# pbenner/kmerLr

Hardware: NVIDIA B200
Metric: kmer_sequences_per_sec (higher is better)
Workload: dtype f64

## Files before the change

kmerlr_b200/csrc/abi.cu:

```cuda
#include <cmath>
#include <map>
#include <mutex>
#include <unordered_map>
#include <vector>

#include "common.cuh"

namespace kl {

namespace {
Ctx g_ctx;
std::mutex g_mutex;
std::unordered_map<uint64_t, std::shared_ptr<Object>> g_objects;
uint64_t g_next = 1;
thread_local std::string g_error;
}

Ctx &ctx() { return g_ctx; }

namespace {
std::multimap<size_t, void *> g_free_blocks;
std::unordered_map<void *, size_t> g_block_size;
constexpr size_t ARENA_GRAIN = (size_t)2 << 20;
}
// ... 32 lines not shown
  KL_CUDA(cudaEventSynchronize(g_ctx.staging_ev));
  if (bytes > g_ctx.staging_bytes) {
    if (g_ctx.staging) KL_CUDA(cudaFreeHost(g_ctx.staging));
    g_ctx.staging = nullptr; g_ctx.staging_bytes = 0;
    const size_t want = (bytes + ARENA_GRAIN - 1) / ARENA_GRAIN * ARENA_GRAIN;
    KL_CUDA(cudaMallocHost(&g_ctx.staging, want));
    g_ctx.staging_bytes = want;
  }
  return g_ctx.staging;
}

namespace {
struct ProfRec { std::string name; cudaEvent_t e0, e1; };
std::vector<ProfRec> g_prof_pending;
std::vector<cudaEvent_t> g_prof_pool;
std::unordered_map<std::string, std::pair<double, int64_t>> g_prof_totals;
cudaEvent_t prof_event() {
  if (!g_prof_pool.empty()) { cudaEvent_t e = g_prof_pool.back(); g_prof_pool.pop_back(); return e; }
  cudaEvent_t e;
  KL_CUDA(cudaEventCreate(&e));
  return e;
}
void prof_resolve() {
  if (g_prof_pending.empty()) return;
  KL_CUDA(cudaStreamSynchronize(g_ctx.stream));
  for (auto &r : g_prof_pending) {
    float ms = 0.f;
    KL_CUDA(cudaEventElapsedTime(&ms, r.e0, r.e1));
    auto &t = g_prof_totals[r.name];
    t.first += ms; t.second += 1;
    g_prof_pool.push_back(r.e0); g_prof_pool.push_back(r.e1);
  }
  g_prof_pending.clear();
}
}
void profile_begin(const char *name) {
  if (g_prof_pending.size() > 8192) prof_resolve();
  ProfRec r{name, prof_event(), prof_event()};
  KL_CUDA(cudaEventRecord(r.e0, g_ctx.stream));
  g_prof_pending.push_back(r);
}
void profile_end() { KL_CUDA(cudaEventRecord(g_prof_pending.back().e1, g_ctx.stream)); }

void require_ready() {
  if (!g_ctx.ready) fail(KMERLR_ERR_NOGPU, "kmerlr_init() has not succeeded: no usable sm_100 GPU (there is no CPU fallback)");
}

uint64_t register_object(std::shared_ptr<Object> o) {
  uint64_t h = g_next++;
// ... 424 lines not shown
```

kmerlr_b200/csrc/common.cuh:

```cuda
#pragma once

#include <cuda_runtime.h>
#include <stdint.h>

#include <chrono>
#include <cstdio>
#include <cstdlib>
#include <cstring>
#include <memory>
#include <string>
#include <vector>

#include "../../include/kmerlr_b200.h"

namespace kl {

struct Error {
  int code;
  std::string msg;
};

[[noreturn]] inline void fail(int code, const std::string &msg) { throw Error{code, msg}; }

#define KL_CUDA(expr)                                                                              \
  do {                                                                                             \
    cudaError_t _e = (expr);                                                                       \
    if (_e != cudaSuccess)                                                                         \
      ::kl::fail(KMERLR_ERR_CUDA, std::string(#expr) + ": " + cudaGetErrorString(_e) + " (" +      \
                                      __FILE__ + ":" + std::to_string(__LINE__) + ")");            \
  } while (0)

#define KL_REQUIRE(cond, msg)                                                                      \
  do {                                                                                             \
// ... 37 lines not shown
  cudaEvent_t copy_ev[CTX_COPY_EVENTS] = {nullptr};
  cudaEvent_t ev0 = nullptr, ev1 = nullptr;
  void *staging = nullptr;
  size_t staging_bytes = 0;
  cudaEvent_t staging_ev = nullptr;
  std::vector<std::shared_ptr<const Numbering>> numbering;
  int64_t launches = 0;
  double last_ms = 0.0;
  bool profiling = false;
  bool implicit_ok = true;
  int super_len = -1;
  int hot_cols = 6144;
  int fused_ticket = 8;
  void *comm = nullptr;
  int rank = 0, world = 1;
  PeerBox *peer = nullptr;
  bool p2p_ok = true;
  bool p2p_allreduce = false;
  int feed_growth = 135;
  int small_long = -1;
  int persist_bps = 0;
  bool coop_supported = true;
  bool coop_ok = true;
};
Ctx &ctx();
void require_ready();

void profile_begin(const char *name);
void profile_end();

#define KL_LAUNCH(kernel, grid, block, smem, ...)                                                  \
  do {                                                                                             \
    if (::kl::ctx().profiling) ::kl::profile_begin(#kernel);                                       \
    kernel<<<(grid), (block), (smem), ::kl::ctx().stream>>>(__VA_ARGS__);                          \
    if (::kl::ctx().profiling) ::kl::profile_end();                                                \
    ::kl::ctx().launches++;                                                                        \
    KL_CUDA(cudaGetLastError());                                                                   \
  } while (0)

inline void sync_stream() { KL_CUDA(cudaStreamSynchronize(ctx().stream)); }

void *host_staging(size_t bytes);
inline void host_staging_done() { KL_CUDA(cudaEventRecord(ctx().staging_ev, ctx().stream)); }

struct Trace {
  bool on;
  std::chrono::steady_clock::time_point t0, last;
  const char *what;
  explicit Trace(const char *w) : what(w) {
    static int env = -1;
    if (env < 0) { const char *e = getenv("KMERLR_TRACE"); env = (e && *e == '1') ? 1 : 0; }
    on = env == 1;
    if (on) t0 = last = std::chrono::steady_clock::now();
  }
  void mark(const char *phase, bool sync = true) {
    if (!on) return;
    if (sync) cudaStreamSynchronize(ctx().stream);
    auto t = std::chrono::steady_clock::now();
    fprintf(stderr, "[trace %s] %-28s %8.3f ms (total %8.3f)\n", what, phase,
            std::chrono::duration<double, std::milli>(t - last).count(),
            std::chrono::duration<double, std::milli>(t - t0).count());
    last = t;
  }
// ... 289 lines not shown
```

kmerlr_b200/csrc/extract.cu:

```cuda
#include <cmath>

#include "extract_kernel.cuh"

namespace kl {

namespace {

using namespace xk;

__global__ void pack_kernel(const uint8_t *__restrict__ seq, const int64_t *__restrict__ off,
                            const int64_t *__restrict__ blk, int64_t n, int64_t total_blocks, int64_t w0, int64_t w1,
                            uint32_t *__restrict__ bits2, uint16_t *__restrict__ inv16) {
  int64_t w = w0 + (int64_t)blockIdx.x * blockDim.x + threadIdx.x;
  if (w >= w1) return;
  const int64_t b = w >> 2;
  int64_t g = (int64_t)((double)b * (double)n / (double)total_blocks);
  g = g < 0 ? 0 : (g > n - 1 ? n - 1 : g);
  int64_t lo, hi, stepw = 1;
  if (blk[g] <= b) {
    lo = g; hi = g + 1;
    while (hi < n && blk[hi] <= b) { lo = hi; stepw <<= 1; hi = hi + stepw < n ? hi + stepw : n; }
  } else {
    hi = g; lo = g - 1;
    while (lo > 0 && blk[lo] > b) { hi = lo; stepw <<= 1; lo = lo - stepw > 0 ? lo - stepw : 0; }
// ... 501 lines not shown
  LI.M = cfg.M; LI.N = cfg.N; LI.op = P.op;
  for (int k = cfg.M; k <= cfg.N + 1; k++) LI.level_off[k] = P.level_off[k];
  std::shared_ptr<const Numbering> num;
  if (n_frozen > 0) {
    frozen_bits.assign((size_t)nw, 0u);
    uint64_t prev = 0;
    for (int64_t j = 0; j < n_frozen; j++) {
      int k = frozen_k[j];
      KL_REQUIRE(k >= cfg.M && k <= cfg.N && frozen_code[j] < (1ull << (2 * k)), "frozen class outside [M,N]");
      uint64_t id = (uint64_t)P.level_off[k] + frozen_code[j];
      KL_REQUIRE(j == 0 || id > prev, "frozen class list must be sorted by (k, code) without duplicates");
      prev = id;
      frozen_bits[id >> 5] |= 1u << (id & 31);
    }
    auto F = std::make_shared<Numbering>();
    F->M = cfg.M; F->N = cfg.N; F->op = P.op; F->nw = nw; F->count = (uint32_t)n_frozen;
    F->bits.alloc((size_t)nw); F->rank.alloc((size_t)nw + 1);
    F->bits.upload(frozen_bits.data(), (size_t)nw);
    number_set(*F);
    num = F;
  } else {
    num = numbering_all(LI, nw);
  }
  DevBuf<unsigned long long> tot(9);
  tot.zero();
  bitmap.zero();
  DevBuf<uint32_t> full(1);
  full.zero();
  P.full = full.p; P.nb_words = nw;
  P.st_id = out->col.p; P.st_cnt = P.binarize ? dummy_cnt.p : out->val_u32.p; P.rowcnt = out->rowcnt.p;
  P.bitmap = bitmap.p; P.nbx = num->nbx.p; P.filter = n_frozen > 0; P.stats = tot.p + 1;
  P.mark = n_frozen == 0;
  DevBuf<uint32_t> lowbits, rowdup;
  if (hybrid) {
    P.events = 1;
    P.low_words = P.t_lo <= P.t_hi ? (int)((P.tl_cnt + 31) / 32) : 0;
    if (P.low_words) { lowbits.alloc((size_t)s.n * P.low_words); P.lowbits = lowbits.p; }
    rowdup.alloc((size_t)s.n);
    P.rowdup = rowdup.p;
  }
  DevBuf<uint32_t> ovf;
  P.ovf_stride = nbl * (s.max_len > 0 ? s.max_len : 1);
  if (nbl && (!P.binarize || hybrid) && s.n > 0) {
    ovf.alloc((size_t)ctx().sm_count * 64 * (size_t)P.ovf_stride);
    P.ovf = ovf.p;
  }
  tr.mark("alloc");

  if (s.n > 0) {
    const int nchunks = feed ? feed->nchunks : 1;
    DevBuf<uint32_t> ticket((size_t)nchunks);
    ticket.zero();
    const bool two_streams = feed && nchunks > 1;
    DevBuf<uint32_t> ovf2;
    if (two_streams && P.ovf) ovf2.alloc((size_t)ctx().sm_count * 64 * (size_t)P.ovf_stride);
    struct StreamSwap {
      cudaStream_t saved;
      explicit StreamSwap(cudaStream_t run) : saved(ctx().stream) { ctx().stream = run; }
      ~StreamSwap() { ctx().stream = saved; }
    };
    if (two_streams) {
      KL_CUDA(cudaEventRecord(ctx().join_ev[0], ctx().stream));
      KL_CUDA(cudaStreamWaitEvent(ctx().alt_stream, ctx().join_ev[0], 0));
    }
    uint32_t *const ovf_even = P.ovf;
    for (int c = 0; c < nchunks; c++) {
      StreamSwap on((two_streams && (c & 1)) ? ctx().alt_stream : ctx().stream);
      P.ovf = (two_streams && (c & 1) && ovf_even) ? ovf2.p : ovf_even;
      P.ticket = ticket.p + c;
      const int64_t r0 = feed ? feed->row[c] : 0, r1 = feed ? feed->row[c + 1] : s.n;
      if (feed) feed->feed(*seqs, c);
      P.row0 = r0; P.n = r1;
      switch (E) {
        case 0: launch_extract<0>(P); break;
        case 2: launch_extract<2>(P); break;
        case 4: launch_extract<4>(P); break;
        case 8: launch_extract<8>(P); break;
        case 16: launch_extract<16>(P); break;
        case 32: launch_extract<32>(P); break;
        default: launch_extract<64>(P); break;
      }
    }
    P.ovf = ovf_even;
    if (two_streams) {
      KL_CUDA(cudaEventRecord(ctx().join_ev[1], ctx().alt_stream));
      KL_CUDA(cudaStreamWaitEvent(ctx().stream, ctx().join_ev[1], 0));
    }
    P.row0 = 0; P.n = s.n;
  }
  tr.mark("extract_kernel");
  unsigned long long *const gres = tot.p + 6;
  if (sharded) {
    const int64_t xw = n_frozen == 0 ? nw : 0, per = xw + 6;
    DevBuf<uint32_t> mine((size_t)per), all((size_t)(per * ctx().world));
    KL_LAUNCH(pack_exchange, (unsigned)((xw + 256) / 256), 256, 0, bitmap.p, xw, (unsigned long long)s.n, tot.p + 1, mine.p);
    comm_allgather_bytes(mine.p, all.p, per * 4);
    KL_LAUNCH(merge_exchange, (unsigned)((xw + 256) / 256), 256, 0, all.p, ctx().world, xw, bitmap.p, gres);
  }
  {
    int64_t blocks = ((s.n > nw ? s.n : nw) + 255) / 256;
    if (blocks > 4 * ctx().sm_count) blocks = 4 * ctx().sm_count;
    KL_LAUNCH(extract_totals, (unsigned)(blocks ? blocks : 1), 256, 0, out->rowcnt.p, s.n, bitmap.p,
              n_frozen == 0 ? num->bits.p : (const uint32_t *)nullptr, nw, tot.p);
  }
  DevBuf<int64_t> evptr;
  if (hybrid) {
    evptr.alloc((size_t)s.n + 1);
    exclusive_scan_u32_to_i64(rowdup.p, evptr.p, s.n);
    KL_CUDA(cudaMemcpyAsync(tot.p + 4, evptr.p + s.n, sizeof(int64_t), cudaMemcpyDeviceToDevice, ctx().stream));
  }
  uint32_t m32 = num->count;
  out->class_ids.alloc((size_t)(m32 ? m32 : 1));
  KL_LAUNCH(enumerate_bits, (unsigned)((nw + 255) / 256), 256, 0, num->bits.p, num->rank.p, nw, out->class_ids.p);
  unsigned long long *htot = (unsigned long long *)host_staging(9 * sizeof(unsigned long long));
  tot.download(htot, 9);
  host_staging_done();
  sync_stream();
  out->nnz = (int64_t)htot[0];
  const unsigned long long hstats[2] = {htot[1], htot[2]}, hres[3] = {htot[6], htot[7], htot[8]};
  const bool hdiffer = htot[3] != 0;
  const int64_t n_events = (int64_t)htot[4];
  int64_t nn = s.n;
  if (sharded) {
    nn = (int64_t)hres[0];
    out->maxsq = (double)hres[1]; out->vmax = (double)hres[2];
    out->has_maxsq = out->has_vmax = true;
  }
  out->n_global = nn;
  out->has_local_stats = true;
  out->local_maxsq = (double)hstats[0]; out->local_vmax = (double)hstats[1];
  tr.mark("sizes");
  if (hdiffer) {
    auto obs = std::make_shared<Numbering>();
    obs->M = cfg.M; obs->N = cfg.N; obs->op = P.op; obs->nw = nw;
    obs->rank.alloc((size_t)nw + 1);
    {
// ... 82 lines not shown
```

kmerlr_b200/csrc/extract_kernel.cuh:

```cuda
#pragma once

#include <type_traits>

#include "common.cuh"

namespace kl {
namespace xk {

#ifndef KL_X_OLDPOS
#define KL_X_OLDPOS 1
#endif
#ifndef KL_X_WALK
#define KL_X_WALK 1
#endif
#ifndef KL_X_TKPRE
#define KL_X_TKPRE 0
#endif
#ifndef KL_X_TLPIPE
#define KL_X_TLPIPE 1
#endif
#ifndef KL_X_MARKSKIP
#define KL_X_MARKSKIP 1
#endif
constexpr uint32_t SENT = 0xFFFFFFFFu;
// ... 801 lines not shown
    if (mk && ++groups == next_check) {
      next_check *= 2;
      __syncthreads();
      flush_marks();
      __threadfence();
      __syncthreads();
      int missing = 0;
      for (int64_t i = threadIdx.x; i < P.nb_words; i += blockDim.x)
        missing |= (__ldg(P.nbx + i).x & ~*(volatile const uint32_t *)(P.bitmap + i)) != 0u;
      if (!__syncthreads_or(missing)) {
        mk = 0;
        if (threadIdx.x == 0) *(volatile uint32_t *)P.full = 1u;
      } else if (__syncthreads_or(threadIdx.x == 0 && *(volatile uint32_t *)P.full != 0u)) {
        mk = 0;
      }
    }
  }
  __syncthreads();
  if (mk) flush_marks();
}

template <int E, int OPT, bool EV>
void launch_extract_op(const XParams &P) {
  KL_CUDA(cudaFuncSetAttribute((extract_kernel<E, OPT, EV>), cudaFuncAttributeMaxDynamicSharedMemorySize, 227 * 1024));
  int best_wpb = 0, best_per_sm = 0;
  for (int wpb = ext_threads(E) / 32; wpb >= 1; wpb--) {
    size_t smem = ((size_t)P.obs_words + (size_t)wpb * P.warp_words) * sizeof(uint32_t);
    if (smem > (size_t)227 * 1024) continue;
    int per_sm = 0;
    KL_CUDA(cudaOccupancyMaxActiveBlocksPerMultiprocessor(&per_sm, (extract_kernel<E, OPT, EV>), 32 * wpb, smem));
    if (per_sm * wpb > best_per_sm * best_wpb) { best_wpb = wpb; best_per_sm = per_sm; }
  }
  KL_REQUIRE(best_wpb > 0, "sequence too long for the shared-memory working set of one warp");
  const int wpb = best_wpb;
  size_t smem = ((size_t)P.obs_words + (size_t)wpb * P.warp_words) * sizeof(uint32_t);
  int64_t blocks = (int64_t)ctx().sm_count * best_per_sm;
  int64_t need = (P.n - P.row0 + wpb - 1) / wpb;
  if (blocks > need) blocks = need;
  if (blocks < 1) blocks = 1;
  KL_LAUNCH((extract_kernel<E, OPT, EV>), (unsigned)blocks, 32 * wpb, smem, P);
}

template <int E>
void launch_extract(const XParams &P) {
  if (P.events) {
    if (P.op == 1) launch_extract_op<E, 1, true>(P);
    else launch_extract_op<E, -1, true>(P);
  } else {
    if (P.op == 1) launch_extract_op<E, 1, false>(P);
    else launch_extract_op<E, -1, false>(P);
  }
}

// ... 5 lines not shown
```

kmerlr_b200/csrc/logistic.cu:

```cuda
#include <cooperative_groups.h>

#include "common.cuh"

#include <cmath>

namespace kl {

namespace {

constexpr int RED_BLOCKS = 256;

struct PgState {
  long long iter;
  int done;
  int first;
  double delta, loss_old, loss_new, lossval;
  int error;
};

__device__ __forceinline__ int64_t ind2sub(int64_t n, int64_t k1, int64_t k2) {
  return n + (n * (n - 1) / 2) - (n - k1) * ((n - k1) - 1) / 2 + k2 - k1;
}

template <typename VT>
// ... 185 lines not shown
                                                             unsigned long long *__restrict__ H, unsigned int *ticket,
                                                             const PgState *st) {
  if (st && st->done == 1) return;
  const uint32_t u = blockIdx.x * blockDim.x + threadIdx.x;
  if (level == P.N) {
    if (u < (1u << (2 * P.S))) {
      const unsigned long long h = H[P.sup0 + u];
      const uint32_t maskN = (1u << (2 * P.N)) - 1u;
      if (h)
        for (int t = 0; t < P.c; t++) atomicAdd(H + P.fo[P.N] + ((u >> (2 * (P.S - P.N - t))) & maskN), h);
    }
  } else if (level >= P.Mlo && u < (1u << (2 * level))) {
    const unsigned long long *c = H + P.fo[level + 1] + 4ull * u;
    H[P.fo[level] + u] += c[0] + c[1] + c[2] + c[3];
  }
  if (tail_top < P.Mlo) return;
  __shared__ int s_last;
  __threadfence();
  __syncthreads();
  if (threadIdx.x == 0) s_last = atomicAdd(ticket, 1u) == gridDim.x - 1 ? 1 : 0;
  __syncthreads();
  if (!s_last) return;
  __threadfence();
  for (int j = tail_top; j >= P.Mlo; j--) {
    for (uint32_t v = threadIdx.x; v < (1u << (2 * j)); v += blockDim.x) {
      const unsigned long long *c = H + P.fo[j + 1] + 4ull * v;
      H[P.fo[j] + v] = __ldcg(H + P.fo[j] + v) + __ldcg(c) + __ldcg(c + 1) + __ldcg(c + 2) + __ldcg(c + 3);
    }
    __syncthreads();
  }
  if (threadIdx.x == 0) *ticket = 0u;
}

__global__ void imp_build_low(const uint32_t *__restrict__ lowcol, int low_words, int lwp,
                              const double *__restrict__ theta, double *__restrict__ lowtab, const PgState *st) {
  if (st && st->done == 1) return;
  const int e = blockIdx.x * blockDim.x + threadIdx.x;
  if (e >= 128 * lwp) return;
  const int l = e % lwp, v = (e / lwp) & 15, i = e / (16 * lwp);
  double s = 0.0;
  if (l < low_words)
    for (int b = 0; b < 4; b++)
      if ((v >> b) & 1) {
        const uint32_t col = lowcol[l * 32 + 4 * i + b];
        if (col != NOCOL) s += theta[col + 1];
      }
  lowtab[e] = s;
}

constexpr uint32_t IMP_NOIDX = 0xFFFFFFFFu, IMP_SINGLES = 0xFFFFFFFEu;
// ... 1166 lines not shown
  const int e = scale_exponent(cmax * (vmax > 0.0 ? vmax : 1.0)), e0 = scale_exponent(cmax * std::fmax(vmax, 1.0));
  wk.scale = std::ldexp(1.0, e);
  wk.inv_scale = std::ldexp(1.0, -e);
  wk.scale0 = std::ldexp(1.0, e0);
  wk.inv_scale0 = std::ldexp(1.0, -e0);
}

bool use_implicit(const Matrix &M) {
  static int env = -1;
  if (env < 0) { const char *e = getenv("KMERLR_IMPLICIT"); env = (e && *e == '0') ? 0 : 1; }
  if (!(env == 1 && ctx().implicit_ok && M.imp)) return false;
  return M.imp->binarized ? M.vt == VAL_ONE : M.vt == VAL_U32;
}

int super_length(int N) {
  int S = ctx().super_len;
  if (S < 0) S = N <= 8 ? 10 : IMP_SUPER_MAX;
  if (S > IMP_SUPER_MAX) S = IMP_SUPER_MAX;
  return S < N ? N : S;
}

template <int CACHE, bool BIN>
void launch_imp_pass(const ImpParams &P, const ImpArgs &A, size_t smem) {
  if (smem > 48 * 1024)
    KL_CUDA(cudaFuncSetAttribute((imp_pass<CACHE, BIN>), cudaFuncAttributeMaxDynamicSharedMemorySize, (int)smem));
  const int64_t blocks = (A.n + A.rpb - 1) / A.rpb;
  KL_LAUNCH((imp_pass<CACHE, BIN>), (unsigned)blocks, 256, smem, P, A);
}

void launch_implicit(Matrix &M, Work &wk, const double cw[2], const PgState *st, int scatter) {
  KL_INVARIANT(wk.scale == wk.scale0);
  const Implicit &I = *M.imp;
  const SeqSet &S = *I.seqs;
  ImpParams P{};
  P.M = I.M; P.N = I.N; P.op = I.op; P.Mlo = I.Mlo;
  for (int k = 0; k < 16; k++) { P.level_off[k] = I.level_off[k]; P.fo[k] = I.fo[k]; }
  const bool levels = I.Mlo <= I.N;
  wk.F = nullptr;
  P.S = levels ? super_length(I.N) : I.N;
  P.c = P.S - I.N + 1;
  const int64_t tlev = levels ? I.fo[I.N + 1] : 0, tsup = P.c > 1 ? (int64_t)1 << (2 * P.S) : 0, total = tlev + tsup;
  P.sup0 = P.c > 1 ? (uint32_t)tlev : I.fo[I.N];
  if (wk.T.n < (size_t)(total ? total : 1)) { wk.T.alloc((size_t)(total ? total : 1)); wk.H.alloc((size_t)(total ? total : 1)); }
  if (scatter && total) KL_CUDA(cudaMemsetAsync(wk.H.p, 0, (size_t)total * sizeof(unsigned long long), ctx().stream));
  if (levels) {
    KL_LAUNCH(imp_build_T, (unsigned)((tlev + 255) / 256), 256, 0, P, I.num->bits.p, I.num->rank.p, wk.theta.p, wk.T.p, tlev, st);
    if (P.c > 1) KL_LAUNCH(imp_build_TS, (unsigned)((tsup + 255) / 256), 256, 0, P, wk.T.p, st);
  }
// ... 37 lines not shown
  if (P.c > 1) steps[nsteps++] = I.N;
  for (int j = I.N - 1; j > small_top && j >= I.Mlo; j--) steps[nsteps++] = j;
  if (nsteps == 0 && small_top >= I.Mlo) steps[nsteps++] = -1;
  for (int s = 0; s < nsteps; s++) {
    const int j = steps[s];
    const int64_t items = j == I.N ? tsup : (j < 0 ? 1 : (int64_t)1 << (2 * j));
    KL_LAUNCH(imp_fold, (unsigned)((items + IMP_FOLD_THREADS - 1) / IMP_FOLD_THREADS), IMP_FOLD_THREADS, 0, P, j,
              s == nsteps - 1 ? small_top : -1, wk.H.p, wk.tickets.p, st);
  }
  wk.P = P;
  wk.F = wk.H.p;
}

template <typename VT>
void launch_fused(Matrix &M, Work &wk, const double cw[2], const PgState *st, int scatter = 1) {
  if (scatter) KL_CUDA(cudaMemsetAsync(wk.G.p, 0, (size_t)(M.m + 2 + PEER_MAX_WORLD) * sizeof(unsigned long long), ctx().stream));
  if (M.n > 0) {
    if (use_implicit(M)) {
      launch_implicit(M, wk, cw, st, scatter);
    } else {
      int hot = ctx().hot_cols;
      if (hot > M.m) hot = (int)M.m;
      const size_t smem = (size_t)hot * 8;
      KL_CUDA(cudaFuncSetAttribute(fused_kernel<VT>, cudaFuncAttributeMaxDynamicSharedMemorySize, HOT_COLS_MAX * 8));
      const int tk = ctx().fused_ticket;
      if (tk > 0) {
        unsigned long long *ticket = wk.G.p + M.m + 1 + PEER_MAX_WORLD;
        KL_CUDA(cudaMemsetAsync(ticket, 0, sizeof(unsigned long long), ctx().stream));
        int per_sm = 0;
        KL_CUDA(cudaOccupancyMaxActiveBlocksPerMultiprocessor(&per_sm, fused_kernel<VT>, 256, smem));
        if (per_sm < 1) per_sm = 1;
        int64_t blocks = (int64_t)ctx().sm_count * per_sm, need = (M.n + 8 * tk - 1) / (8 * tk);
        if (blocks > need) blocks = need;
        KL_LAUNCH((fused_kernel<VT>), (unsigned)blocks, 256, smem, M.rows(), M.col.p, csr_val<VT>(M), M.n, M.m, wk.theta.p,
                  M.labels.p, cw[0], cw[1], 1.0 / (double)M.n_global, wk.scale, wk.scale0, wk.G.p, wk.lossterm.p, st, scatter, hot, tk,
                  ticket);
      } else {
        int rpb = FUSED_RPB;
        while ((M.n + rpb - 1) / rpb > 0x7fffffffLL) rpb *= 2;
        KL_LAUNCH((fused_kernel<VT>), (unsigned)((M.n + rpb - 1) / rpb), 256, smem, M.rows(), M.col.p, csr_val<VT>(M), M.n,
                  M.m, wk.theta.p, M.labels.p, cw[0], cw[1], 1.0 / (double)M.n_global, wk.scale, wk.scale0, wk.G.p, wk.lossterm.p, st,
                  scatter, hot, rpb, (unsigned long long *)nullptr);
      }
    }
  }
}

void alloc_work(const Matrix &M, int64_t ntheta, Work &wk) {
  wk.theta.alloc((size_t)ntheta);
  wk.w.alloc((size_t)(M.n ? M.n : 1));
  wk.lossterm.alloc((size_t)(M.n ? M.n : 1));
  wk.g.alloc((size_t)ntheta);
  wk.G.alloc((size_t)M.m + 2 + PEER_MAX_WORLD);
// ... 50 lines not shown
  Work wk; alloc_work(M, ntheta, wk);
  set_scale(M, wk, cw);
  wk.theta.upload(theta, (size_t)ntheta);
  wk.g.zero();
  dispatch_vt(M, [&](auto *tag) {
    using VT = typename std::remove_pointer<decltype(tag)>::type;
    if (!cooc) {
      launch_fused<VT>(M, wk, cw, nullptr);
      if (wk.F) launch_pass_tail(M, wk, nullptr, ntheta, NAN, 0, 0.0);
      if (M.sharded) comm_allreduce_sum_i64_fast((int64_t *)wk.G.p, M.m + 1);
    } else {
      PairTerms terms;
      collect_pair_terms(M, theta, ntheta, cooc, terms);
      launch_rows<VT, 2>(M, wk.theta.p, cooc, cw, wk.w.p, wk.lossterm.p, nullptr, &terms);
      ensure_csc(M);
      KL_CUDA(cudaMemsetAsync(wk.G.p, 0, (size_t)(M.m + 1) * sizeof(unsigned long long), ctx().stream));
      if (M.n > 0)
        KL_LAUNCH((scatter_w<VT>), warp_grid(M.n, 256), 256, 0, M.rows(), M.col.p, csr_val<VT>(M), M.n, wk.w.p,
                  wk.scale, wk.scale0, wk.G.p);
      if (M.sharded) comm_allreduce_sum_i64((int64_t *)wk.G.p, M.m + 1);
      if (M.m > 1) {
        const int ntile = (int)((M.m + PAIR_T - 1) / PAIR_T);
        const size_t smem = (size_t)PAIR_CH * PAIR_T * sizeof(double) + (size_t)8 * PAIR_CH * (sizeof(double) + sizeof(unsigned short));
        KL_CUDA(cudaFuncSetAttribute(pairs_gradient<VT>, cudaFuncAttributeMaxDynamicSharedMemorySize, (int)smem));
        KL_LAUNCH((pairs_gradient<VT>), (unsigned)((int64_t)ntile * (ntile + 1) / 2), 256, smem, M.colptr.p, M.crow.p,
                  csc_val<VT>(M), M.m, M.n, ntile, wk.w.p, wk.g.p);
        if (M.sharded) {
          comm_allgather_f64(wk.g.p, wk.gathered.p, ntheta);
          KL_LAUNCH(sum_ranks, (unsigned)((ntheta + 255) / 256), 256, 0, wk.gathered.p, ctx().world, ntheta, wk.g.p);
        }
      }
    }
  });
  KL_LAUNCH(finalize_g, (unsigned)((M.m + 1 + 255) / 256), 256, 0, wk.G.p, M.m + 1, wk.inv_scale, wk.inv_scale0, wk.g.p);
  if (!std::isnan(lambda) && lambda != 0.0)
    KL_LAUNCH(add_l1_sign, (unsigned)((ntheta + 255) / 256), 256, 0, wk.theta.p, wk.g.p, ntheta, lambda);
  if (g_host) wk.g.download(g_host, (size_t)ntheta);
  sync_stream();
  if (M.sharded) comm_check_peer_errors();
  if (g_dev) *g_dev = std::move(wk.g);
}

double loss(Matrix &M, const double *theta, int64_t ntheta, const double cw[2], double lambda, int cooc) {
  require_ready();
  check_theta(M, ntheta, cooc);
  KL_REQUIRE(M.has_labels, "loss: the matrix has no labels (kmerlr_matrix_set_labels)");
  if (M.n_global == 0) return 0.0;
// ... 40 lines not shown
  const double inv_n = 1.0 / (double)M.n_global;
  const bool small = ntheta <= SMALL_MAX_THETA && !use_implicit(M);
  const bool p2p = M.sharded && ctx().peer && ctx().p2p_ok;
  bool persistent = small && ctx().coop_ok && (!M.sharded || p2p);
  bool long_rows = persistent && M.nnz > 0 && (ctx().small_long >= 1 || (ctx().small_long < 0 && M.nnz >= 4 * M.n));
  DevBuf<double> wbuf;
  bool packed = false;
  if (long_rows) { ensure_sliced(M); ensure_csc(M); packed = ensure_packed(M); wbuf.alloc((size_t)M.n); }
  int long_mode = long_rows ? 1 : 0;
  size_t dyn_smem = 0;
  const bool want_block = long_rows && packed && (ctx().small_long == 2 || ctx().small_long < 0);
  const int64_t BATCH = persistent ? 4096 : (small ? 256 : 16);
  int small_blocks = 0;
  DevBuf<double> blockloss;
  DevBuf<unsigned int> counter;
  DevBuf<unsigned long long> G3;
  if (small) {
    int64_t nb = (int64_t)ctx().sm_count * SMALL_BLOCKS_PER_SM, need = (M.n + 63) / 64;
    if (persistent) {
      auto resident = [&](int mode, size_t smem) {
        int per_sm = 0;
        dispatch_vt(M, [&](auto *tag) {
          using VT = typename std::remove_pointer<decltype(tag)>::type;
          if (smem > 16 * 1024)
            KL_CUDA(cudaFuncSetAttribute(persistent_kernel<VT>(M.sharded, mode), cudaFuncAttributeMaxDynamicSharedMemorySize, 32 * 1024));
          KL_CUDA(cudaOccupancyMaxActiveBlocksPerMultiprocessor(&per_sm, persistent_kernel<VT>(M.sharded, mode), PERSIST_THREADS, smem));
        });
        if (ctx().persist_bps > 0 && ctx().persist_bps < per_sm) per_sm = ctx().persist_bps;
        return per_sm;
      };
      if (want_block) {
        int per_sm = resident(2, 0);
        for (int round = 0; round < 4 && per_sm >= 1; round++) {
          int64_t g = (int64_t)ctx().sm_count * per_sm;
          if (g > need) g = need;
          const size_t smem = (size_t)((M.n + g - 1) / g + 1) * sizeof(double);
          const int p2 = smem <= 32 * 1024 ? resident(2, smem) : 0;
          if (p2 >= per_sm) { dyn_smem = smem; break; }
          per_sm = p2;
        }
        if (per_sm >= 1 && dyn_smem > 0) {
          int64_t g = (int64_t)ctx().sm_count * per_sm;
          if (g > need) g = need;
          if (ensure_blockview(M, (int)g)) { long_mode = 2; nb = (int64_t)ctx().sm_count * per_sm; }
          else dyn_smem = 0;
        } else dyn_smem = 0;
      }
      if (long_mode != 2 && long_rows && ctx().small_long < 0 && M.nnz < 8 * M.n) { long_rows = false; long_mode = 0; }
      if (long_mode != 2) {
// ... 124 lines not shown
```

kmerlr_b200/csrc/matrix.cu:

```cuda
#include "common.cuh"

#include <cmath>

namespace kl {

namespace {

constexpr int RS_THREADS = 256;
constexpr int RS_GROUPS = 32;
constexpr int RS_WARP_ITEMS = 32 * RS_GROUPS;
constexpr int RS_TILE = (RS_THREADS / 32) * RS_WARP_ITEMS;

__global__ void __launch_bounds__(RS_THREADS) radix_hist(const uint32_t *__restrict__ keys, int64_t nnz, int shift,
                                                         uint32_t *__restrict__ hist, int64_t ntiles) {
  __shared__ uint32_t h[256];
  h[threadIdx.x] = 0;
  __syncthreads();
  int64_t base = (int64_t)blockIdx.x * RS_TILE;
#pragma unroll 8
  for (int i = 0; i < RS_TILE / RS_THREADS; i++) {
    int64_t p = base + (int64_t)i * RS_THREADS + threadIdx.x;
    if (p < nnz) atomicAdd(&h[(keys[p] >> shift) & 255u], 1u);
  }
  __syncthreads();
// ... 524 lines not shown
  const int64_t nnz = M.nnz, ntiles = (nnz + RS_TILE - 1) / RS_TILE;
  int bits = 1;
  while (((int64_t)1 << bits) < M.m) bits++;
  const int passes = (bits + 7) / 8;
  Trace tr("csc");
  DevBuf<uint32_t> hist((size_t)(256 * ntiles));
  DevBuf<int64_t> offs((size_t)(256 * ntiles) + 1);
  DevBuf<uint32_t> kA((size_t)nnz), kB(passes > 1 ? (size_t)nnz : 1), rA(passes > 1 ? (size_t)nnz : 1),
      rB(passes > 2 ? (size_t)nnz : 1);
  DevBuf<VT> vA(val && passes > 1 ? (size_t)nnz : 1), vB(val && passes > 2 ? (size_t)nnz : 1);
  const uint32_t *kin = M.col.p, *rin = nullptr;
  const VT *vin = val;
  tr.mark("alloc");
  for (int ps = 0; ps < passes; ps++) {
    const bool last = ps == passes - 1;
    uint32_t *kout = (ps & 1) ? kB.p : kA.p;
    if (passes == 1) kout = kA.p;
    uint32_t *rout = last ? M.crow.p : ((ps & 1) ? rB.p : rA.p);
    VT *vout = val ? (last ? cval : ((ps & 1) ? vB.p : vA.p)) : nullptr;
    KL_LAUNCH(radix_hist, (unsigned)ntiles, RS_THREADS, 0, kin, nnz, 8 * ps, hist.p, ntiles);
    exclusive_scan_u32_to_i64(hist.p, offs.p, 256 * ntiles);
    const size_t smem = (size_t)RS_TILE * (8 + (val ? sizeof(VT) : 0));
    if (ps == 0) {
      KL_CUDA(cudaFuncSetAttribute(radix_scatter<VT, true>, cudaFuncAttributeMaxDynamicSharedMemorySize, (int)smem));
      KL_LAUNCH((radix_scatter<VT, true>), (unsigned)ntiles, RS_THREADS, smem, kin, rin, M.rowptr.p, M.n, vin, nnz, 8 * ps,
                offs.p, ntiles, kout, rout, vout);
    } else {
      KL_CUDA(cudaFuncSetAttribute(radix_scatter<VT, false>, cudaFuncAttributeMaxDynamicSharedMemorySize, (int)smem));
      KL_LAUNCH((radix_scatter<VT, false>), (unsigned)ntiles, RS_THREADS, smem, kin, rin, M.rowptr.p, M.n, vin, nnz, 8 * ps,
                offs.p, ntiles, kout, rout, vout);
    }
    kin = kout; rin = rout; vin = vout;
    tr.mark("pass");
  }
  KL_LAUNCH(lower_bounds, (unsigned)((M.m + 1 + 255) / 256), 256, 0, kin, nnz, M.m, M.colptr.p);
  sync_stream();
}

void ensure_csc(Matrix &M) {
  if (M.has_csc) return;
  matrix_compact(M);
  M.colptr.alloc((size_t)M.m + 1);
  M.crow.alloc((size_t)(M.nnz ? M.nnz : 1));
  if (M.m == 0 || M.n == 0 || M.nnz == 0) {
    M.colptr.zero();
  } else if (M.vt == VAL_U32) {
    M.cval_u32.alloc((size_t)(M.nnz ? M.nnz : 1));
    build_csc<uint32_t>(M, M.val_u32.p, M.cval_u32.p);
  } else if (M.vt == VAL_F64) {
    M.cval_f64.alloc((size_t)(M.nnz ? M.nnz : 1));
    build_csc<double>(M, M.val_f64.p, M.cval_f64.p);
// ... 281 lines not shown
```

kmerlr_b200/csrc/score.cu:

```cuda
#include "common.cuh"
#include "kmer_class.cuh"

#include <cmath>

namespace kl {

namespace {

constexpr uint32_t HEMPTY = 0xFFFFFFFFu;

struct DevModel {
  int M, N, op, binarize, summary;
  int n_classes, n_features, n_members;
  uint32_t hmask;
  uint32_t levels;
  ClassRule rule;
  uint32_t level_off[16];
  uint32_t hit_cap;
  uint32_t hit_size;
  const uint32_t *hkeys;
  const int32_t *hvals;
  const int32_t *feat;
  const double *theta;
  const double *cweight;
// ... 482 lines not shown
        const int wt_bytes = hs_smem && d.wtab ? SCORE_WT * 8 : 0;
        int64_t TP = (200 * 1024 - hs_smem * 8 - wt_bytes) / (8 * nlev) - 1;
        if (TP > 16384) TP = 16384;
        const bool scratch = TP < W + step;
        if (scratch) {
          const int64_t more = std::max<int64_t>(0, std::min<int64_t>(W, 16384) / step - 1);
          TP = W + more * step;
          KL_REQUIRE(TP < ((int64_t)1 << 30), "score_windows: window too large");
        }
        int64_t starts = (TP - W) / step + 1;
        std::vector<LinearTile> tiles;
        for (int64_t r = 0; r < s.n; r++) {
          int64_t nw = win_off[r + 1] - win_off[r];
          for (int64_t w0 = 0; w0 < nw; w0 += starts) tiles.push_back(LinearTile{r, w0 * step});
        }
        DevBuf<LinearTile> dt(tiles.size() ? tiles.size() : 1);
        dt.upload(tiles.data(), tiles.size());
        const int64_t grid_cap = scratch ? (int64_t)ctx().sm_count : INT64_MAX;
        DevBuf<double> qbuf;
        if (scratch) qbuf.alloc((size_t)std::min<int64_t>(grid_cap, (int64_t)tiles.size()) * nlev * (size_t)(TP + 1));
        size_t smem = (scratch ? 0 : (size_t)nlev * (size_t)(TP + 1) * sizeof(double)) + (size_t)hs_smem * 8 + (size_t)wt_bytes;
        auto kern = gen ? (scratch ? score_linear<true, true> : score_linear<true, false>)
                        : (scratch ? score_linear<false, true> : score_linear<false, false>);
        KL_CUDA(cudaFuncSetAttribute(kern, cudaFuncAttributeMaxDynamicSharedMemorySize, (int)smem));
        const int nch = feed ? feed->chunks() : 1;
        size_t t0 = 0;
        for (int c = 0; c < nch; c++) {
          const int64_t r0 = feed ? feed->first_row(c) : 0, r1 = feed ? feed->first_row(c + 1) : s.n;
          if (feed && mi == 0) feed->feed(c);
          size_t t1 = t0;
          while (t1 < tiles.size() && tiles[t1].region < r1) t1++;
          if (t1 > t0) {
            const int64_t nt = (int64_t)(t1 - t0);
            const unsigned grid = (unsigned)std::min<int64_t>(nt, grid_cap);
            const int64_t stride = layout == 1 ? step : (int64_t)1;
            if (!gen && !scratch)
              KL_LAUNCH((score_linear<false, false>), grid, SCORE_THREADS, smem, dmodels.p, 0, mi > 0 ? 1 : 0, s.len.p,
                        s.blk.p, s.bits2.p, s.inv16.p, dt.p + t0, nt, dslot.p, W, step, (int)TP, mi, hs_smem, stride,
                        qbuf.p, outbuf->val_f64.p);
            else if (!gen)
              KL_LAUNCH((score_linear<false, true>), grid, SCORE_THREADS, smem, dmodels.p, 0, mi > 0 ? 1 : 0, s.len.p,
                        s.blk.p, s.bits2.p, s.inv16.p, dt.p + t0, nt, dslot.p, W, step, (int)TP, mi, hs_smem, stride,
                        qbuf.p, outbuf->val_f64.p);
            else if (!scratch)
              KL_LAUNCH((score_linear<true, false>), grid, SCORE_THREADS, smem, dmodels.p, 0, mi > 0 ? 1 : 0, s.len.p,
                        s.blk.p, s.bits2.p, s.inv16.p, dt.p + t0, nt, dslot.p, W, step, (int)TP, mi, hs_smem, stride,
                        qbuf.p, outbuf->val_f64.p);
// ... 14 lines not shown
            copied_home = true;
          }
        }
        sync_stream();
      }
      if (copied_home) KL_CUDA(cudaStreamSynchronize(ctx().alt_stream));
    } else if (any_hits) {
      if (feed) feed->feed(-1);
      int64_t tab = 32;
      for (auto &h : hm) tab = std::max<int64_t>(tab, (int64_t)h->d.hit_size);
      tab = (tab + 31) / 32 * 32;
      const int64_t per_warp = 2 * tab * (int64_t)sizeof(uint32_t);
      int64_t warps = std::min<int64_t>((int64_t)ctx().sm_count * 64, std::max<int64_t>(32, ((int64_t)512 << 20) / per_warp));
      warps = std::min<int64_t>(warps, (total_windows + 3) / 4 * 4);
      const int64_t blocks = (warps + 3) / 4;
      DevBuf<uint32_t> tabs((size_t)(blocks * 4 * 2 * tab));
      KL_CUDA(cudaMemsetAsync(tabs.p, 0xFF, (size_t)(blocks * 4 * tab) * sizeof(uint32_t), ctx().stream));
      KL_CUDA(cudaMemsetAsync(tabs.p + blocks * 4 * tab, 0, (size_t)(blocks * 4 * tab) * sizeof(uint32_t), ctx().stream));
      KL_LAUNCH(score_hits, (unsigned)blocks, 128, 0, dmodels.p, n_models, s.blk.p, s.bits2.p, s.inv16.p, s.n, dwin.p,
                dslot.p, total_windows, W, step, layout == 1 ? step : (int64_t)1, tabs.p, tab, outbuf->val_f64.p);
    } else {
      if (feed) feed->feed(-1);
      size_t smem = (size_t)4 * (size_t)max_classes * sizeof(uint32_t);
      KL_CUDA(cudaFuncSetAttribute(score_generic, cudaFuncAttributeMaxDynamicSharedMemorySize, (int)smem));
      int64_t blocks = (total_windows + 3) / 4, cap = (int64_t)ctx().sm_count * 16;
      if (blocks > cap) blocks = cap;
      KL_LAUNCH(score_generic, (unsigned)blocks, 128, smem, dmodels.p, n_models, s.len.p, s.blk.p, s.bits2.p,
                s.inv16.p, s.n, dwin.p, dslot.p, total_windows, W, step, max_classes, layout == 1 ? step : (int64_t)1,
                outbuf->val_f64.p);
    }
  }
  else if (feed) feed->feed(-1);
  if (out_host && !copied_home) outbuf->val_f64.download(out_host, (size_t)total_slots);
  sync_stream();
  if (out_dev) *out_dev = outbuf;
}

}
```

Before: 58.85 million.

## Cache kernel attributes and occupancy, merge small buffers, overlap enumeration, fuse tail reduction

Caches the cudaFuncSetAttribute and occupancy queries in the context so repeated launches skip those driver calls. Folds the ticket and full-flag allocations into the existing stats buffer to save allocations and memsets. Moves class-id enumeration onto the alternate stream so it overlaps with extraction. Rewrites the histogram tail reduction in logistic to handle two levels per pass with vector loads and warp shuffles, and changes profiling resolution to per-event sync. The caches assume attributes only ever need to grow and that occupancy results are stable.

```diff
diff --git a/kmerlr_b200/csrc/abi.cu b/kmerlr_b200/csrc/abi.cu
--- a/kmerlr_b200/csrc/abi.cu
+++ b/kmerlr_b200/csrc/abi.cu
@@ -78,9 +78,8 @@
   return e;
 }
 void prof_resolve() {
-  if (g_prof_pending.empty()) return;
-  KL_CUDA(cudaStreamSynchronize(g_ctx.stream));
   for (auto &r : g_prof_pending) {
+    KL_CUDA(cudaEventSynchronize(r.e1));
     float ms = 0.f;
     KL_CUDA(cudaEventElapsedTime(&ms, r.e0, r.e1));
     auto &t = g_prof_totals[r.name];
diff --git a/kmerlr_b200/csrc/common.cuh b/kmerlr_b200/csrc/common.cuh
--- a/kmerlr_b200/csrc/common.cuh
+++ b/kmerlr_b200/csrc/common.cuh
@@ -7,8 +7,10 @@
 #include <cstdio>
 #include <cstdlib>
 #include <cstring>
+#include <map>
 #include <memory>
 #include <string>
+#include <tuple>
 #include <vector>
 
 #include "../../include/kmerlr_b200.h"
@@ -92,6 +94,8 @@
   int persist_bps = 0;
   bool coop_supported = true;
   bool coop_ok = true;
+  std::map<const void *, size_t> smem_limits;
+  std::map<std::tuple<const void *, int, size_t>, int> occupancy;
 };
 Ctx &ctx();
 void require_ready();
@@ -109,6 +113,22 @@
   } while (0)
 
 inline void sync_stream() { KL_CUDA(cudaStreamSynchronize(ctx().stream)); }
+
+inline void smem_limit(const void *func, size_t bytes) {
+  size_t &have = ctx().smem_limits[func];
+  if (bytes <= have) return;
+  KL_CUDA(cudaFuncSetAttribute(func, cudaFuncAttributeMaxDynamicSharedMemorySize, (int)bytes));
+  have = bytes;
+}
+inline int blocks_per_sm(const void *func, int threads, size_t smem) {
+  const auto key = std::make_tuple(func, threads, smem);
+  auto it = ctx().occupancy.find(key);
+  if (it != ctx().occupancy.end()) return it->second;
+  int n = 0;
+  KL_CUDA(cudaOccupancyMaxActiveBlocksPerMultiprocessor(&n, func, threads, smem));
+  ctx().occupancy.emplace(key, n);
+  return n;
+}
 
 void *host_staging(size_t bytes);
 inline void host_staging_done() { KL_CUDA(cudaEventRecord(ctx().staging_ev, ctx().stream)); }
diff --git a/kmerlr_b200/csrc/extract.cu b/kmerlr_b200/csrc/extract.cu
--- a/kmerlr_b200/csrc/extract.cu
+++ b/kmerlr_b200/csrc/extract.cu
@@ -547,12 +547,11 @@
   } else {
     num = numbering_all(LI, nw);
   }
-  DevBuf<unsigned long long> tot(9);
+  const int nchunks = s.n > 0 && feed ? feed->nchunks : 1;
+  DevBuf<unsigned long long> tot((size_t)(10 + (nchunks + 1) / 2));
   tot.zero();
   bitmap.zero();
-  DevBuf<uint32_t> full(1);
-  full.zero();
-  P.full = full.p; P.nb_words = nw;
+  P.full = reinterpret_cast<uint32_t *>(tot.p + 9); P.nb_words = nw;
   P.st_id = out->col.p; P.st_cnt = P.binarize ? dummy_cnt.p : out->val_u32.p; P.rowcnt = out->rowcnt.p;
   P.bitmap = bitmap.p; P.nbx = num->nbx.p; P.filter = n_frozen > 0; P.stats = tot.p + 1;
   P.mark = n_frozen == 0;
@@ -572,10 +571,11 @@
   }
   tr.mark("alloc");
 
+  uint32_t m32 = num->count;
+  out->class_ids.alloc((size_t)(m32 ? m32 : 1));
+  bool listed = false;
   if (s.n > 0) {
-    const int nchunks = feed ? feed->nchunks : 1;
-    DevBuf<uint32_t> ticket((size_t)nchunks);
-    ticket.zero();
+    uint32_t *const ticket = reinterpret_cast<uint32_t *>(tot.p + 10);
     const bool two_streams = feed && nchunks > 1;
     DevBuf<uint32_t> ovf2;
     if (two_streams && P.ovf) ovf2.alloc((size_t)ctx().sm_count * 64 * (size_t)P.ovf_stride);
@@ -584,15 +584,13 @@
       explicit StreamSwap(cudaStream_t run) : saved(ctx().stream) { ctx().stream = run; }
       ~StreamSwap() { ctx().stream = saved; }
     };
-    if (two_streams) {
-      KL_CUDA(cudaEventRecord(ctx().join_ev[0], ctx().stream));
-      KL_CUDA(cudaStreamWaitEvent(ctx().alt_stream, ctx().join_ev[0], 0));
-    }
+    KL_CUDA(cudaEventRecord(ctx().join_ev[0], ctx().stream));
+    KL_CUDA(cudaStreamWaitEvent(ctx().alt_stream, ctx().join_ev[0], 0));
     uint32_t *const ovf_even = P.ovf;
     for (int c = 0; c < nchunks; c++) {
       StreamSwap on((two_streams && (c & 1)) ? ctx().alt_stream : ctx().stream);
       P.ovf = (two_streams && (c & 1) && ovf_even) ? ovf2.p : ovf_even;
-      P.ticket = ticket.p + c;
+      P.ticket = ticket + c;
       const int64_t r0 = feed ? feed->row[c] : 0, r1 = feed ? feed->row[c + 1] : s.n;
       if (feed) feed->feed(*seqs, c);
       P.row0 = r0; P.n = r1;
@@ -607,10 +605,13 @@
       }
     }
     P.ovf = ovf_even;
-    if (two_streams) {
-      KL_CUDA(cudaEventRecord(ctx().join_ev[1], ctx().alt_stream));
-      KL_CUDA(cudaStreamWaitEvent(ctx().stream, ctx().join_ev[1], 0));
-    }
+    {
+      StreamSwap on(ctx().alt_stream);
+      KL_LAUNCH(enumerate_bits, (unsigned)((nw + 255) / 256), 256, 0, num->bits.p, num->rank.p, nw, out->class_ids.p);
+      listed = true;
+    }
+    KL_CUDA(cudaEventRecord(ctx().join_ev[1], ctx().alt_stream));
+    KL_CUDA(cudaStreamWaitEvent(ctx().stream, ctx().join_ev[1], 0));
     P.row0 = 0; P.n = s.n;
   }
   tr.mark("extract_kernel");
@@ -634,9 +635,8 @@
     exclusive_scan_u32_to_i64(rowdup.p, evptr.p, s.n);
     KL_CUDA(cudaMemcpyAsync(tot.p + 4, evptr.p + s.n, sizeof(int64_t), cudaMemcpyDeviceToDevice, ctx().stream));
   }
-  uint32_t m32 = num->count;
-  out->class_ids.alloc((size_t)(m32 ? m32 : 1));
-  KL_LAUNCH(enumerate_bits, (unsigned)((nw + 255) / 256), 256, 0, num->bits.p, num->rank.p, nw, out->class_ids.p);
+  if (!listed)
+    KL_LAUNCH(enumerate_bits, (unsigned)((nw + 255) / 256), 256, 0, num->bits.p, num->rank.p, nw, out->class_ids.p);
   unsigned long long *htot = (unsigned long long *)host_staging(9 * sizeof(unsigned long long));
   tot.download(htot, 9);
   host_staging_done();
diff --git a/kmerlr_b200/csrc/extract_kernel.cuh b/kmerlr_b200/csrc/extract_kernel.cuh
--- a/kmerlr_b200/csrc/extract_kernel.cuh
+++ b/kmerlr_b200/csrc/extract_kernel.cuh
@@ -847,13 +847,13 @@
 
 template <int E, int OPT, bool EV>
 void launch_extract_op(const XParams &P) {
-  KL_CUDA(cudaFuncSetAttribute((extract_kernel<E, OPT, EV>), cudaFuncAttributeMaxDynamicSharedMemorySize, 227 * 1024));
+  const void *kern = (const void *)extract_kernel<E, OPT, EV>;
+  smem_limit(kern, 227 * 1024);
   int best_wpb = 0, best_per_sm = 0;
   for (int wpb = ext_threads(E) / 32; wpb >= 1; wpb--) {
     size_t smem = ((size_t)P.obs_words + (size_t)wpb * P.warp_words) * sizeof(uint32_t);
     if (smem > (size_t)227 * 1024) continue;
-    int per_sm = 0;
-    KL_CUDA(cudaOccupancyMaxActiveBlocksPerMultiprocessor(&per_sm, (extract_kernel<E, OPT, EV>), 32 * wpb, smem));
+    const int per_sm = blocks_per_sm(kern, 32 * wpb, smem);
     if (per_sm * wpb > best_per_sm * best_wpb) { best_wpb = wpb; best_per_sm = per_sm; }
   }
   KL_REQUIRE(best_wpb > 0, "sequence too long for the shared-memory working set of one warp");
diff --git a/kmerlr_b200/csrc/logistic.cu b/kmerlr_b200/csrc/logistic.cu
--- a/kmerlr_b200/csrc/logistic.cu
+++ b/kmerlr_b200/csrc/logistic.cu
@@ -231,10 +231,36 @@
   __syncthreads();
   if (!s_last) return;
   __threadfence();
-  for (int j = tail_top; j >= P.Mlo; j--) {
-    for (uint32_t v = threadIdx.x; v < (1u << (2 * j)); v += blockDim.x) {
-      const unsigned long long *c = H + P.fo[j + 1] + 4ull * v;
-      H[P.fo[j] + v] = __ldcg(H + P.fo[j] + v) + __ldcg(c) + __ldcg(c + 1) + __ldcg(c + 2) + __ldcg(c + 3);
+  for (int j = tail_top; j >= P.Mlo; j -= 2) {
+    const bool two = j - 1 >= P.Mlo;
+    const uint32_t pairs = 1u << (2 * (j + 1) - 1);
+    const ulonglong2 *src = reinterpret_cast<const ulonglong2 *>(H + P.fo[j + 1]);
+    constexpr int U = 4;
+    for (uint32_t t0 = threadIdx.x; (t0 & ~31u) < pairs; t0 += U * blockDim.x) {
+      ulonglong2 x[U];
+      unsigned long long hj[U], hv[U];
+#pragma unroll
+      for (int k = 0; k < U; k++) {
+        const uint32_t t = t0 + k * blockDim.x;
+        x[k] = t < pairs ? __ldcg(src + t) : make_ulonglong2(0ull, 0ull);
+        hj[k] = t < pairs && (t & 1u) == 0u ? __ldcg(H + P.fo[j] + (t >> 1)) : 0ull;
+        hv[k] = two && t < pairs && (t & 7u) == 0u ? __ldcg(H + P.fo[j - 1] + (t >> 3)) : 0ull;
+      }
+#pragma unroll
+      for (int k = 0; k < U; k++) {
+        const uint32_t t = t0 + k * blockDim.x;
+        if ((t & ~31u) >= pairs) break;
+        unsigned long long f = x[k].x + x[k].y;
+        f += __shfl_xor_sync(0xffffffffu, f, 1);
+        f += hj[k];
+        if (t < pairs && (t & 1u) == 0u) H[P.fo[j] + (t >> 1)] = f;
+        if (two) {
+          unsigned long long g = (t & 1u) == 0u ? f : 0ull;
+          g += __shfl_xor_sync(0xffffffffu, g, 2);
+          g += __shfl_xor_sync(0xffffffffu, g, 4);
+          if (t < pairs && (t & 7u) == 0u) H[P.fo[j - 1] + (t >> 3)] = g + hv[k];
+        }
+      }
     }
     __syncthreads();
   }
@@ -1447,8 +1473,7 @@
 
 template <int CACHE, bool BIN>
 void launch_imp_pass(const ImpParams &P, const ImpArgs &A, size_t smem) {
-  if (smem > 48 * 1024)
-    KL_CUDA(cudaFuncSetAttribute((imp_pass<CACHE, BIN>), cudaFuncAttributeMaxDynamicSharedMemorySize, (int)smem));
+  if (smem > 48 * 1024) smem_limit((const void *)imp_pass<CACHE, BIN>, smem);
   const int64_t blocks = (A.n + A.rpb - 1) / A.rpb;
   KL_LAUNCH((imp_pass<CACHE, BIN>), (unsigned)blocks, 256, smem, P, A);
 }
@@ -1532,13 +1557,12 @@
       int hot = ctx().hot_cols;
       if (hot > M.m) hot = (int)M.m;
       const size_t smem = (size_t)hot * 8;
-      KL_CUDA(cudaFuncSetAttribute(fused_kernel<VT>, cudaFuncAttributeMaxDynamicSharedMemorySize, HOT_COLS_MAX * 8));
+      smem_limit((const void *)fused_kernel<VT>, HOT_COLS_MAX * 8);
       const int tk = ctx().fused_ticket;
       if (tk > 0) {
         unsigned long long *ticket = wk.G.p + M.m + 1 + PEER_MAX_WORLD;
         KL_CUDA(cudaMemsetAsync(ticket, 0, sizeof(unsigned long long), ctx().stream));
-        int per_sm = 0;
-        KL_CUDA(cudaOccupancyMaxActiveBlocksPerMultiprocessor(&per_sm, fused_kernel<VT>, 256, smem));
+        int per_sm = blocks_per_sm((const void *)fused_kernel<VT>, 256, smem);
         if (per_sm < 1) per_sm = 1;
         int64_t blocks = (int64_t)ctx().sm_count * per_sm, need = (M.n + 8 * tk - 1) / (8 * tk);
         if (blocks > need) blocks = need;
@@ -1635,7 +1659,7 @@
       if (M.m > 1) {
         const int ntile = (int)((M.m + PAIR_T - 1) / PAIR_T);
         const size_t smem = (size_t)PAIR_CH * PAIR_T * sizeof(double) + (size_t)8 * PAIR_CH * (sizeof(double) + sizeof(unsigned short));
-        KL_CUDA(cudaFuncSetAttribute(pairs_gradient<VT>, cudaFuncAttributeMaxDynamicSharedMemorySize, (int)smem));
+        smem_limit((const void *)pairs_gradient<VT>, smem);
         KL_LAUNCH((pairs_gradient<VT>), (unsigned)((int64_t)ntile * (ntile + 1) / 2), 256, smem, M.colptr.p, M.crow.p,
                   csc_val<VT>(M), M.m, M.n, ntile, wk.w.p, wk.g.p);
         if (M.sharded) {
@@ -1722,9 +1746,8 @@
         int per_sm = 0;
         dispatch_vt(M, [&](auto *tag) {
           using VT = typename std::remove_pointer<decltype(tag)>::type;
-          if (smem > 16 * 1024)
-            KL_CUDA(cudaFuncSetAttribute(persistent_kernel<VT>(M.sharded, mode), cudaFuncAttributeMaxDynamicSharedMemorySize, 32 * 1024));
-          KL_CUDA(cudaOccupancyMaxActiveBlocksPerMultiprocessor(&per_sm, persistent_kernel<VT>(M.sharded, mode), PERSIST_THREADS, smem));
+          if (smem > 16 * 1024) smem_limit(persistent_kernel<VT>(M.sharded, mode), 32 * 1024);
+          per_sm = blocks_per_sm(persistent_kernel<VT>(M.sharded, mode), PERSIST_THREADS, smem);
         });
         if (ctx().persist_bps > 0 && ctx().persist_bps < per_sm) per_sm = ctx().persist_bps;
         return per_sm;
diff --git a/kmerlr_b200/csrc/matrix.cu b/kmerlr_b200/csrc/matrix.cu
--- a/kmerlr_b200/csrc/matrix.cu
+++ b/kmerlr_b200/csrc/matrix.cu
@@ -570,11 +570,11 @@
     exclusive_scan_u32_to_i64(hist.p, offs.p, 256 * ntiles);
     const size_t smem = (size_t)RS_TILE * (8 + (val ? sizeof(VT) : 0));
     if (ps == 0) {
-      KL_CUDA(cudaFuncSetAttribute(radix_scatter<VT, true>, cudaFuncAttributeMaxDynamicSharedMemorySize, (int)smem));
+      smem_limit((const void *)radix_scatter<VT, true>, smem);
       KL_LAUNCH((radix_scatter<VT, true>), (unsigned)ntiles, RS_THREADS, smem, kin, rin, M.rowptr.p, M.n, vin, nnz, 8 * ps,
                 offs.p, ntiles, kout, rout, vout);
     } else {
-      KL_CUDA(cudaFuncSetAttribute(radix_scatter<VT, false>, cudaFuncAttributeMaxDynamicSharedMemorySize, (int)smem));
+      smem_limit((const void *)radix_scatter<VT, false>, smem);
       KL_LAUNCH((radix_scatter<VT, false>), (unsigned)ntiles, RS_THREADS, smem, kin, rin, M.rowptr.p, M.n, vin, nnz, 8 * ps,
                 offs.p, ntiles, kout, rout, vout);
     }
diff --git a/kmerlr_b200/csrc/score.cu b/kmerlr_b200/csrc/score.cu
--- a/kmerlr_b200/csrc/score.cu
+++ b/kmerlr_b200/csrc/score.cu
@@ -528,7 +528,7 @@
         size_t smem = (scratch ? 0 : (size_t)nlev * (size_t)(TP + 1) * sizeof(double)) + (size_t)hs_smem * 8 + (size_t)wt_bytes;
         auto kern = gen ? (scratch ? score_linear<true, true> : score_linear<true, false>)
                         : (scratch ? score_linear<false, true> : score_linear<false, false>);
-        KL_CUDA(cudaFuncSetAttribute(kern, cudaFuncAttributeMaxDynamicSharedMemorySize, (int)smem));
+        smem_limit((const void *)kern, smem);
         const int nch = feed ? feed->chunks() : 1;
         size_t t0 = 0;
         for (int c = 0; c < nch; c++) {
@@ -589,7 +589,7 @@
     } else {
       if (feed) feed->feed(-1);
       size_t smem = (size_t)4 * (size_t)max_classes * sizeof(uint32_t);
-      KL_CUDA(cudaFuncSetAttribute(score_generic, cudaFuncAttributeMaxDynamicSharedMemorySize, (int)smem));
+      smem_limit((const void *)score_generic, smem);
       int64_t blocks = (total_windows + 3) / 4, cap = (int64_t)ctx().sm_count * 16;
       if (blocks > cap) blocks = cap;
       KL_LAUNCH(score_generic, (unsigned)blocks, 128, smem, dmodels.p, n_models, s.len.p, s.blk.p, s.bits2.p,
```

Result: no change. 59.13 million, median of 6 (+0.5%).
